# starlingonearth/MASt3R-SLAM-Quality-dualTSDF

Hardware: AMD Instinct MI355X
Metric: SLAM frames/sec (infer+match+TSDF+GN) @512x384 (higher is better)
Workload: dtype bf16

## Files before the change

### include/mslam_hip.h

```cpp
#ifndef MSLAM_HIP_H
#define MSLAM_HIP_H

#include <stddef.h>
#include <stdint.h>

#ifdef __cplusplus
extern "C" {
#endif

#define MSLAM_OK 0
#define MSLAM_EINVAL (-1)
#define MSLAM_EHIP (-2)
#define MSLAM_ENOMEM (-3)
#define MSLAM_ENODEV (-4)

const char* mslam_last_error(void);
int mslam_abi_version(void);
int mslam_device_check(void);


int mslam_iter_proj(const float* rays_img_with_grad, const float* pts_3d_norm,
                    const float* p_init, float* p_new, uint8_t* converged, int b, int h, int w,
                    int n, int max_iter, float lambda_init, float cost_thresh, void* stream);

int mslam_refine_matches(const uint16_t* D11, const uint16_t* D21, const int64_t* p1,
                         int64_t* p1_new, int b, int h, int w, int n, int fdim, int radius,
                         int dilation_max, void* stream);

int mslam_prep_iter_proj(const float* X11, const float* X21, const int64_t* idx_init,
                         float* rays_img_with_grad, float* pts_3d_norm, float* p_init, int b, int h,
                         int w, void* stream);

int mslam_match_occlusion(const float* X11, const float* X21, const float* p, int64_t* p1,
                          uint8_t* valid, int b, int h, int w, float dist_thresh, void* stream);

int mslam_pixel_to_lin(const int64_t* p1, int64_t* idx, int b, int n, int w, void* stream);

size_t mslam_gn_workspace_bytes(int num_poses, int num_edges, int num_points, int local_edges);

int mslam_gauss_newton_rays(float* Twc, const float* Xs, const float* Cs, const int64_t* ii,
                            const int64_t* jj, const int64_t* idx_ii2jj, const uint8_t* valid_match,
                            const float* Q, int num_poses, int num_points, int num_edges,
                            float sigma_ray, float sigma_dist, float C_thresh, float Q_thresh,
                            int max_iter, float delta_thresh, float* dx, void* workspace,
                            size_t workspace_bytes, void* stream);

int mslam_gauss_newton_calib(float* Twc, const float* Xs, const float* Cs, const float* K,
                             const int64_t* ii, const int64_t* jj, const int64_t* idx_ii2jj,
                             const uint8_t* valid_match, const float* Q, int num_poses, int num_points,
                             int num_edges, int height, int width, int pixel_border, float z_eps,
                             float sigma_pixel, float sigma_depth, float C_thresh, float Q_thresh,
                             int max_iter, float delta_thresh, float* dx, void* workspace,
                             size_t workspace_bytes, void* stream);

int mslam_gauss_newton_points(float* Twc, const float* Xs, const float* Cs, const int64_t* ii,
                              const int64_t* jj, const int64_t* idx_ii2jj, const uint8_t* valid_match,
                              const float* Q, int num_poses, int num_points, int num_edges,
                              float sigma_point, float C_thresh, float Q_thresh, int max_iter,
                              float delta_thresh, float* dx, void* workspace, size_t workspace_bytes,
                              void* stream);

int mslam_gn_begin(const int64_t* ii, const int64_t* jj, int num_poses, int num_edges, int num_points,
                   void* workspace, size_t workspace_bytes, void* stream);
int mslam_gn_compact(const float* Xs, const float* Cs, const int64_t* idx_ii2jj, const uint8_t* valid_match,
                     const float* Q, int num_poses, int num_points, int num_edges, int edge_begin,
                     int edge_count, float C_thresh, float Q_thresh, void* workspace, size_t workspace_bytes,
                     void* stream);
int mslam_gn_compact_at(const float* Xs, const float* Cs, const int64_t* idx_ii2jj, const uint8_t* valid_match,
                        const float* Q, int num_poses, int num_points, int num_edges, int edge_begin, int edge_count,
                        int slot_begin, int range_count, float C_thresh, float Q_thresh, void* workspace,
                        size_t workspace_bytes, void* stream);
int mslam_gn_accumulate(int kind, const float* Twc, const float* K, int num_poses, int num_points,
                        int num_edges, int edge_begin, int edge_count, float sigma_a, float sigma_b,
                        int height, int width, int pixel_border, float z_eps, float* Hs, float* gs,
                        void* workspace, size_t workspace_bytes, void* stream);
int mslam_gn_solve_retract(const float* Hs, const float* gs, int num_poses, int num_edges,
                           int num_points, float* Twc, float* dx, float delta_thresh, void* workspace,
                           size_t workspace_bytes, void* stream);
int mslam_gn_status(int* status4, int num_poses, int num_edges, int num_points, void* workspace,
                    size_t workspace_bytes, void* stream);

int mslam_sim3_act(const float* T, const float* X, float* Y, int num_poses, long long pts_per_pose,
                   int broadcast_pose, void* stream);
int mslam_sim3_op(int op, const float* A, const float* B, float* out, int n, int bcast_a, int bcast_b,
                  void* stream);

size_t mslam_tsdf_table_bytes(uint64_t capacity);
int mslam_tsdf_table_init(void* table, size_t table_bytes, uint64_t capacity, void* stream);

size_t mslam_tsdf_integrate_workspace_bytes(int n_points, double voxel_size, double trunc, double step_scale);
int mslam_tsdf_integrate(void* table, uint64_t capacity, const float* points_world, const double* conf,
                         const float* cam_origin, int n_points, double voxel_size, double trunc,
                         double max_weight, double step_scale, int shard_id, int num_shards,
                         void* workspace, size_t workspace_bytes, void* stream);

int mslam_tsdf_rehash(void* old_table, uint64_t old_capacity, void* new_table, uint64_t new_capacity, void* stream);
int mslam_tsdf_header(void* table, uint64_t capacity, uint32_t* out8_host, void* stream);

int mslam_tsdf_dump(void* table, uint64_t capacity, int64_t* keys, double* tsdf, double* weight,
                    uint32_t max_out, void* stream);

int mslam_tsdf_query(void* table, uint64_t capacity, const float* points, int n, double voxel_size,
                     double min_weight, double* value, double* grad, uint8_t* status, void* stream);

int mslam_tsdf_pose_step(void* table, uint64_t capacity, const float* points, const float* conf, int n,
                         float* pose, int points_in_camera_frame, double voxel_size, double min_weight,
                         double lambda, double damping, int update_pose, double* H_out, double* b_out,
                         int* used_out, void* workspace, size_t workspace_bytes, void* stream);

int mslam_tsdf_lookup7(void* table, uint64_t capacity, const float* points, int n, const float* pose,
                       double voxel_size, double* out, void* stream);
int mslam_tsdf_query_lookup(const double* lookup, int n, double voxel_size, double min_weight, double* value,
                            double* grad, uint8_t* status, void* stream);
int mslam_tsdf_pose_step_lookup(const double* lookup, const float* points, const float* conf, int n, float* pose,
                                int points_in_camera_frame, double voxel_size, double min_weight, double lambda,
                                double damping, int update_pose, double* H_out, double* b_out, int* used_out,
                                void* workspace, size_t workspace_bytes, void* stream);

size_t mslam_tsdf_mesh_workspace_bytes(uint64_t capacity);
int mslam_tsdf_mesh_keys(void* table, uint64_t capacity, double min_weight, int64_t* sort_keys, void* stream);
int mslam_tsdf_mesh_count(void* table, uint64_t capacity, double min_weight, double level, const int64_t* sorted_keys,
                          const int64_t* order, int32_t* counts, void* workspace, size_t workspace_bytes, void* stream);
int mslam_tsdf_mesh_emit(void* table, uint64_t capacity, double voxel_size, double min_weight, double level,
                         const int64_t* sorted_keys, const int64_t* order, const int64_t* vbase, const int64_t* fbase,
                         void* workspace, size_t workspace_bytes, float* vertices, float* normals, int32_t* faces,
                         int64_t n_vertices, int64_t n_faces, void* stream);
int mslam_tsdf_load(void* table, uint64_t capacity, const int64_t* keys, const double* tsdf, const double* weight,
                    int n, void* stream);

size_t mslam_tsdf_render_workspace_bytes(uint64_t capacity);
int mslam_tsdf_render_blocks(void* table, uint64_t capacity, double min_weight, void* workspace, size_t workspace_bytes,
                             void* stream);
int mslam_tsdf_render(void* table, uint64_t capacity, const float* rays, int h, int w, const float* pose8,
                      double voxel_size, double min_weight, double level, double near, double far, double step, int skip,
                      const void* workspace, size_t workspace_bytes, float* range, float* normal, uint8_t* hit,
                      void* stream);

size_t mslam_tsdf_color_bytes(uint64_t capacity);
int mslam_tsdf_color_init(void* color, size_t color_bytes, uint64_t capacity, void* stream);
int mslam_tsdf_integrate_color(void* table, uint64_t capacity, void* color, const float* points_world,
                               const double* conf, const float* rgb, const float* cam_origin, int n_points,
                               double voxel_size, double trunc, double step_scale, void* stream);
int mslam_tsdf_color_rehash(void* old_table, uint64_t old_capacity, const void* old_color, void* new_table,
                            uint64_t new_capacity, void* new_color, void* stream);
int mslam_tsdf_color_dump(void* table, uint64_t capacity, const void* color, const int64_t* keys, int n, uint64_t* sums,
                          void* stream);
int mslam_tsdf_color_load(void* table, uint64_t capacity, void* color, const int64_t* keys, const uint64_t* sums, int n,
                          void* stream);
int mslam_tsdf_color_sample(void* table, uint64_t capacity, const void* color, const float* points, int n, int image_w,
                            double voxel_size, double default_r, double default_g, double default_b, float* out_rgb,
                            uint8_t* out_count, void* stream);

int mslam_mast3r_create(void** handle_out, const int* cfg9_host, void* const* weight_ptrs_host,
                        const long long* weight_numels_host, int n_weights, void* stream);
int mslam_mast3r_destroy(void* handle);
size_t mslam_mast3r_workspace_bytes(void* handle, int batch, int H, int W);

int mslam_mast3r_encode(void* handle, const float* img, int batch, int H, int W, float* feat_out,
                        void* workspace, size_t workspace_bytes, void* stream);

int mslam_mast3r_decode(void* handle, const float* feat1, const float* feat2, int batch, int H, int W,
                        float* X1, float* C1, float* D1, float* Q1, float* X2, float* C2, float* D2,
                        float* Q2, float* dec_last1, float* dec_last2, void* workspace,
                        size_t workspace_bytes, void* stream);

size_t mslam_track_workspace_bytes(int n_points);
int mslam_track_pose(int use_calib, float* T_rel, const float* Xf, const float* Xk, const int64_t* idx_f2k,
                     const float* Qk, const uint8_t* valid, int n_points, const float* K, int width,
                     int height, float sigma_a, float sigma_b, float huber, int pixel_border, float z_eps,
                     int first_iter, int max_iters, float rel_error, float delta_norm, void* status_out, void* workspace,
                     size_t workspace_bytes, void* stream);

size_t mslam_track_prepare_workspace_bytes(int n_points);
int mslam_track_prepare(const int64_t* idx_f2k, const uint8_t* valid_match, const float* Qff, const float* Qkf,
                        const float* Cf_sum, float inv_nf, const float* Ck_sum, float inv_nk, float C_conf, float Q_conf,
                        int n_points, const float* T_WCk, const float* T_WCf, float* Qk, float* Ck_avg,
                        uint8_t* valid_opt, uint8_t* valid_kf, float* T_rel, void* workspace, size_t workspace_bytes,
                        void* stream);
int mslam_track_verdict(const void* prepare_workspace, const void* status, int n_points, float* verdict6, void* stream);
int mslam_track_fuse(const float* T_WCk, const float* T_rel, const float* Xkf, const float* Ckf, const float* X_canon,
                     const float* C, int n_points, float* T_WCf, float* X_new, float* C_new, void* stream);

int mslam_gemm_bf16(const void* A, const void* W, const float* bias, const void* residual_f32, void* out,
                    int M, int N, int K, int act, int out_is_bf16, void* stream);
int mslam_gemm_tile_override(int M, int N, int K, int cfg);
int mslam_gemm_profile_begin(int M, int N, int K, int max_samples);
int mslam_gemm_profile_end(double* avg_us, double* min_us, int* samples);
int mslam_conv2d_nhwc_bf16(const void* in, const void* W, const float* bias, const void* residual_bf16,
                           void* out_bf16, int B, int H, int Wd, int Cin, int Cout, int ks, int stride,
                           int relu_in, int act, void* stream);
int mslam_attention_bf16(const void* Q, const void* K, const void* VT, void* O, int batch, int heads,
                         int nq, int nk, void* stream);
int mslam_layernorm_f32(const float* x, const float* w, const float* b, void* out_bf16, float* out_f32,
                        int rows, int D, float eps, void* stream);

size_t mslam_tsdf_local_workspace_bytes(int n_points);
int mslam_tsdf_local_build(const float* X_world, const float* C, const float* origin, const float* xyz_min,
                           const float* xyz_max, int n_points, int nx, int ny, int nz, double voxel_size,
                           double trunc, float min_confidence, float* tsdf, float* weights, void* workspace,
                           size_t workspace_bytes, void* stream);
int mslam_tsdf_local_raycast(const float* tsdf, int nx, int ny, int nz, const float* xyz_min,
                             const float* xyz_max, const float* X_original, const int64_t* sel_pix, int n_sel,
                             int n_samples, float max_displacement, float* surf, uint8_t* hit, void* stream);

int mslam_quality_reduce_grid(const float* x, const float* y, const uint8_t* valid, int h, int w, int ps, int mode,
                              double c_thr, double q_thr, float* out, void* stream);
int mslam_quality_classify(const float* delta_cov, const float* r, const float* u, int n, float thr_zr, float thr_zu,
                           float thr_dc, int64_t* cls, float* pri, void* stream);

int mslam_room_pair(const float* ki, const float* kj, int batch, int h, int w, int n_frames, double fx, double fy,
                    double cx, double cy, double noise, const double* Wm_3x24, const double* phase_24, float* X1,
                    float* C1, float* D1, float* Q1, float* X2, float* C2, float* D2, float* Q2, void* stream);

int mslam_remap_bilinear_u8(const uint8_t* src, int src_h, int src_w, int channels, const float* mapx,
                            const float* mapy, uint8_t* dst, int dst_h, int dst_w, void* stream);

int mslam_gemm_f64(const void* A, int a_is_f32, const void* B, int b_is_f32, int b_transposed, const double* centre,
                   const double* bias, double* out, int M, int N, int K, void* stream);

int mslam_asmk_aggregate(const float* des, const float* centroids, const int64_t* assign, const int64_t* uniq_words,
                         uint32_t* sig_out, int n_des, int m_assign, int dim, int n_uniq, int n_centroids, void* stream);
int mslam_asmk_search(const int32_t* entry_word, const uint32_t* entry_sig, const int32_t* img_start, int n_images,
                      const int32_t* q_words, const uint32_t* q_sig, int n_q, int sig_words, float similarity_threshold,
                      float alpha, double* scores, void* stream);

#ifdef __cplusplus
}
#endif
#endif
```

### mast3r-slam-quality-dualtsdf_amd/csrc/tracker.hip

```cpp
#include "common.h"
#include "sim3.h"

namespace mslam {

constexpr int kTAcc = 36;

struct TrackState {
  int done;
  int iters;
  int chol_fail;
  float old_cost;
  float last_cost;
  float last_delta_norm;
  float pad0, pad1;
};

struct TrackParams {
  float inv_sigma_a, inv_sigma_b;
  float huber_k;
  const float* K;
  float border_lo, border_hi_u, border_hi_v, z_eps;
  int width;
};

__device__ __forceinline__ float huber_k(float r, float k) {
  const float a = fabsf(r);
  return a < k ? 1.0f : k / a;
}

template <unsigned NZ>
__device__ __forceinline__ void taccum_row(float (&acc)[kTAcc], const float (&x)[7], float w, float err) {
  const float we = w * err;
  int l = 0;
#pragma unroll
  for (int n = 0; n < 7; n++) {
    const float wx = w * x[n];
#pragma unroll
    for (int m = 0; m <= n; m++) {
      if (((NZ >> n) & 1u) && ((NZ >> m) & 1u)) acc[l] = fmaf(wx, x[m], acc[l]);
      l++;
    }
    if ((NZ >> n) & 1u) acc[28 + n] = fmaf(we, x[n], acc[28 + n]);
  }
  acc[35] = fmaf(we, err, acc[35]);
}

template <int CALIB>
__global__ __launch_bounds__(256) void track_accum_kernel(const TrackState* __restrict__ st,
                                                          const float* __restrict__ T,
                                                          const float* __restrict__ Xf, const float* __restrict__ Xk,
                                                          const int64_t* __restrict__ idx, const float* __restrict__ Qk,
                                                          const uint8_t* __restrict__ valid, int n, TrackParams P,
                                                          float* __restrict__ partial) {
  if (st->done) return;
  const Sim3f Tr = sim3_load(T);
  float R[9];
  quat_to_mat(Tr.q, R);
  float acc[kTAcc];
#pragma unroll
  for (int l = 0; l < kTAcc; l++) acc[l] = 0.0f;
  for (int k = blockIdx.x * 256 + threadIdx.x; k < n; k += gridDim.x * 256) {
    const long long j = idx[k];
    const float xf0 = Xf[j * 3], xf1 = Xf[j * 3 + 1], xf2 = Xf[j * 3 + 2];
    const float xk0 = Xk[(size_t)k * 3], xk1 = Xk[(size_t)k * 3 + 1], xk2 = Xk[(size_t)k * 3 + 2];
    const float p0 = Tr.s * (R[0] * xf0 + R[1] * xf1 + R[2] * xf2) + Tr.t[0];
    const float p1 = Tr.s * (R[3] * xf0 + R[4] * xf1 + R[5] * xf2) + Tr.t[1];
    const float p2 = Tr.s * (R[6] * xf0 + R[7] * xf1 + R[8] * xf2) + Tr.t[2];
    const float vq = valid[k] ? sqrtf(Qk[k]) : 0.0f;
    if constexpr (CALIB == 0) {
      const float nk = sqrtf(xk0 * xk0 + xk1 * xk1 + xk2 * xk2), nk_inv = 1.0f / nk;
      const float n2 = p0 * p0 + p1 * p1 + p2 * p2;
      const float np = sqrtf(n2), np_inv = 1.0f / np;
      const float r0 = p0 * np_inv, r1 = p1 * np_inv, r2 = p2 * np_inv;
      const float e0 = r0 - xk0 * nk_inv, e1 = r1 - xk1 * nk_inv, e2 = r2 - xk2 * nk_inv, e3 = np - nk;
      const float sa = P.inv_sigma_a * vq, sb = P.inv_sigma_b * vq;
      const float w0 = huber_k(sa * e0, P.huber_k) * sa * sa, w1 = huber_k(sa * e1, P.huber_k) * sa * sa;
      const float w2 = huber_k(sa * e2, P.huber_k) * sa * sa, w3 = huber_k(sb * e3, P.huber_k) * sb * sb;
      const float n3 = np_inv / n2;
      const float dxx = np_inv - p0 * p0 * n3, dyy = np_inv - p1 * p1 * n3, dzz = np_inv - p2 * p2 * n3;
      const float dxy = -p0 * p1 * n3, dxz = -p0 * p2 * n3, dyz = -p1 * p2 * n3;
      { const float x[7] = {dxx, dxy, dxz, 0.0f, r2, -r1, 0.0f}; taccum_row<0b0110111>(acc, x, w0, e0); }
      { const float x[7] = {dxy, dyy, dyz, -r2, 0.0f, r0, 0.0f}; taccum_row<0b0101111>(acc, x, w1, e1); }
      { const float x[7] = {dxz, dyz, dzz, r1, -r0, 0.0f, 0.0f}; taccum_row<0b0011111>(acc, x, w2, e2); }
      { const float x[7] = {r0, r1, r2, 0.0f, 0.0f, 0.0f, np}; taccum_row<0b1000111>(acc, x, w3, e3); }
    } else {
      const float Pfx = P.K[0], Pfy = P.K[4], Pcx = P.K[2], Pcy = P.K[5];
      const float uk = (float)(k % P.width), vk = (float)(k / P.width);
      const bool valid_meas = xk2 > P.z_eps;
      const float lzk = valid_meas ? logf(xk2) : 0.0f;
      const float zinv = 1.0f / p2;
      const float u = Pfx * p0 * zinv + Pcx, v = Pfy * p1 * zinv + Pcy;
      const bool valid_z = p2 > P.z_eps;
      const bool valid_p = (u > P.border_lo) && (u < P.border_hi_u) && (v > P.border_lo) && (v < P.border_hi_v) && valid_z;
      const float lz = valid_z ? logf(p2) : 0.0f;
      const float gate = (valid_p && valid_meas) ? vq : 0.0f;
      const float e0 = u - (valid_meas ? uk : 0.0f), e1 = v - (valid_meas ? vk : 0.0f), e2 = lz - lzk;
      const float sa = P.inv_sigma_a * gate, sb = P.inv_sigma_b * gate;
      const float w0 = huber_k(sa * e0, P.huber_k) * sa * sa, w1 = huber_k(sa * e1, P.huber_k) * sa * sa;
      const float w2 = huber_k(sb * e2, P.huber_k) * sb * sb;
      const float xz = p0 * zinv, yz = p1 * zinv;
      if (gate > 0.0f) {
        { const float x[7] = {Pfx * zinv, 0.0f, -Pfx * xz * zinv, -Pfx * xz * yz, Pfx * (1.0f + xz * xz), -Pfx * yz, 0.0f};
          taccum_row<0b0111101>(acc, x, w0, e0); }
        { const float x[7] = {0.0f, Pfy * zinv, -Pfy * yz * zinv, -Pfy * (1.0f + yz * yz), Pfy * xz * yz, Pfy * xz, 0.0f};
          taccum_row<0b0111110>(acc, x, w1, e1); }
        { const float x[7] = {0.0f, 0.0f, zinv, yz, -xz, 0.0f, 1.0f}; taccum_row<0b1011100>(acc, x, w2, e2); }
      }
    }
  }
  __shared__ float red[4][kTAcc];
  const int lane = threadIdx.x & 63, wid = threadIdx.x >> 6;
#pragma unroll
  for (int l = 0; l < kTAcc; l++) {
    const float s = wave_sum(acc[l]);
    if (lane == 0) red[wid][l] = s;
  }
  __syncthreads();
  if (threadIdx.x < kTAcc)
    partial[(size_t)blockIdx.x * kTAcc + threadIdx.x] =
        (red[0][threadIdx.x] + red[1][threadIdx.x]) + (red[2][threadIdx.x] + red[3][threadIdx.x]);
}

__global__ __launch_bounds__(64) void track_solve_kernel(TrackState* __restrict__ st, const float* __restrict__ partial,
                                                         int nblk, float* __restrict__ T, float rel_thresh,
                                                         float delta_thresh) {
  if (st->done) return;
  __shared__ double s[kTAcc];
  const int t = threadIdx.x;
  if (t < kTAcc) {
    double a = 0.0;
    for (int k = 0; k < nblk; k++) a += (double)partial[(size_t)k * kTAcc + t];
    s[t] = a;
  }
  __syncthreads();
  if (t != 0) return;
  double H[7][7], g[7];
  int l = 0;
  for (int n = 0; n < 7; n++)
    for (int m = 0; m <= n; m++) { H[n][m] = s[l]; H[m][n] = s[l]; l++; }
  for (int n = 0; n < 7; n++) g[n] = -s[28 + n];
  const float cost = (float)(0.5 * s[35]);
  double L[7][7];
  bool fail = false;
  for (int j = 0; j < 7 && !fail; j++) {
    double d = H[j][j];
    for (int k = 0; k < j; k++) d -= L[j][k] * L[j][k];
    if (!(d > 0.0)) { fail = true; break; }
    L[j][j] = sqrt(d);
    for (int i = j + 1; i < 7; i++) {
      double v = H[i][j];
      for (int k = 0; k < j; k++) v -= L[i][k] * L[j][k];
      L[i][j] = v / L[j][j];
    }
  }
  st->iters += 1;
  st->last_cost = cost;
  if (fail) { st->chol_fail = 1; st->done = 1; return; }
  double y[7], x[7];
  for (int i = 0; i < 7; i++) { double v = g[i]; for (int k = 0; k < i; k++) v -= L[i][k] * y[k]; y[i] = v / L[i][i]; }
  for (int i = 6; i >= 0; i--) { double v = y[i]; for (int k = i + 1; k < 7; k++) v -= L[k][i] * x[k]; x[i] = v / L[i][i]; }
  float tau[7];
  double nn = 0.0;
  for (int i = 0; i < 7; i++) { tau[i] = (float)x[i]; nn += (double)tau[i] * tau[i]; }
  sim3_store(T, sim3_unit(sim3_retr(tau, sim3_load(T))));
  const float delta_norm = (float)sqrt(nn);
  st->last_delta_norm = delta_norm;
  const float old = st->old_cost;
  const float rel_dec = fabsf((old - cost) / old);
  if (rel_dec < rel_thresh || delta_norm < delta_thresh) st->done = 1;
  st->old_cost = cost;
}

__global__ void track_init_kernel(TrackState* st) {
  st->done = 0; st->iters = 0; st->chol_fail = 0; st->old_cost = INFINITY; st->last_cost = 0.0f;
  st->last_delta_norm = 0.0f; st->pad0 = st->pad1 = 0.0f;
}

__device__ __host__ inline size_t prep_partials_bytes(int n) { return (((size_t)((n + 255) / 256) * 8) + 255) & ~(size_t)255; }

__global__ __launch_bounds__(256) void track_prep_kernel(
    const int64_t* __restrict__ idx, const uint8_t* __restrict__ vmatch, const float* __restrict__ Qff,
    const float* __restrict__ Qkf, const float* __restrict__ Cf_sum, float inv_nf, const float* __restrict__ Ck_sum,
    float inv_nk, float C_conf, float Q_conf, int n, const float* __restrict__ T_WCk, const float* __restrict__ T_WCf,
    float* __restrict__ Qk, float* __restrict__ Ck_avg, uint8_t* __restrict__ valid_opt, uint8_t* __restrict__ valid_kf,
    float* __restrict__ T_rel, int2* __restrict__ partial, uint8_t* __restrict__ hit) {
  const int k = blockIdx.x * 256 + threadIdx.x;
  if (k == 0) {
    const Sim3f Ti = sim3_unit(sim3_inv(sim3_load(T_WCk)));
    sim3_store(T_rel, sim3_unit(sim3_mul(Ti, sim3_load(T_WCf))));
  }
  bool opt = false, kf = false;
  if (k < n) {
    const long long j = idx[k];
    const bool vm = vmatch[k] != 0;
    const float q = sqrtf(Qff[j] * Qkf[k]);
    const float cf = Cf_sum[j] * inv_nf;
    const float ck = Ck_sum[k] * inv_nk;
    const bool vq = q > Q_conf;
    opt = vm && (cf > C_conf) && (ck > C_conf) && vq;
    kf = vm && vq;
    Qk[k] = q;
    Ck_avg[k] = ck;
    valid_opt[k] = opt ? 1 : 0;
    valid_kf[k] = kf ? 1 : 0;
    if (vm) hit[j] = 1;
  }
  __shared__ int red[4][2];
  const int c_opt = __popcll(__ballot(opt)), c_kf = __popcll(__ballot(kf));
  if ((threadIdx.x & 63) == 0) { red[threadIdx.x >> 6][0] = c_opt; red[threadIdx.x >> 6][1] = c_kf; }
  __syncthreads();
  if (threadIdx.x == 0)
    partial[blockIdx.x] = make_int2(red[0][0] + red[1][0] + red[2][0] + red[3][0], red[0][1] + red[1][1] + red[2][1] + red[3][1]);
}

__global__ __launch_bounds__(1024) void track_verdict_kernel(const int2* __restrict__ partial, const uint8_t* __restrict__ hit,
                                                             const int* __restrict__ status, int n, float* __restrict__ out) {
  const int t = threadIdx.x;
  int c[3] = {0, 0, 0};
  const int nblk = (n + 255) / 256;
  for (int b = t; b < nblk; b += 1024) { const int2 p = partial[b]; c[0] += p.x; c[1] += p.y; }
  const int n16 = n >> 4;
  for (int v = t; v < n16; v += 1024) {
    const uint4 w = reinterpret_cast<const uint4*>(hit)[v];
    c[2] += __popc(w.x) + __popc(w.y) + __popc(w.z) + __popc(w.w);
  }
  for (int v = (n16 << 4) + t; v < n; v += 1024) c[2] += hit[v];
  __shared__ int red[16][3];
#pragma unroll
  for (int q = 0; q < 3; q++) {
    int s = c[q];
#pragma unroll
    for (int off = 32; off > 0; off >>= 1) s += __shfl_down(s, off, 64);
    if ((t & 63) == 0) red[t >> 6][q] = s;
  }
  __syncthreads();
  if (t != 0) return;
  int tot[3] = {0, 0, 0};
  for (int w = 0; w < 16; w++) { tot[0] += red[w][0]; tot[1] += red[w][1]; tot[2] += red[w][2]; }
  const float inv_n = 1.0f / (float)n;
  out[0] = (float)tot[0] * inv_n;
  out[1] = (float)status[1];
  out[2] = (float)status[2];
  out[3] = (float)tot[1] * inv_n;
  out[4] = (float)tot[2] * inv_n;
  out[5] = (float)status[0];
}

__global__ __launch_bounds__(256) void track_fuse_kernel(const float* __restrict__ T_WCk, const float* __restrict__ T_rel,
                                                         const float* __restrict__ Xkf, const float* __restrict__ Ckf,
                                                         const float* __restrict__ Xc, const float* __restrict__ Cc, int n,
                                                         float* __restrict__ T_WCf, float* __restrict__ Xn,
                                                         float* __restrict__ Cn) {
  const int k = blockIdx.x * 256 + threadIdx.x;
  const Sim3f Tr = sim3_load(T_rel);
  if (k == 0) sim3_store(T_WCf, sim3_unit(sim3_mul(sim3_load(T_WCk), Tr)));
  if (k >= n) return;
  const float x[3] = {Xkf[(size_t)k * 3], Xkf[(size_t)k * 3 + 1], Xkf[(size_t)k * 3 + 2]};
  float y[3];
  sim3_act(Tr, x, y);
  const float c = Cc[k], cn = Ckf[k], den = c + cn;
#pragma unroll
  for (int d = 0; d < 3; d++) Xn[(size_t)k * 3 + d] = ((c * Xc[(size_t)k * 3 + d]) + (cn * y[d])) / den;
  Cn[k] = den;
}

}

using namespace mslam;

extern "C" size_t mslam_track_workspace_bytes(int n_points) {
  (void)n_points;
  return 256 + sizeof(float) * kTAcc * 1024;
}

extern "C" int mslam_track_pose(int use_calib, float* T_rel, const float* Xf, const float* Xk, const int64_t* idx_f2k,
                                const float* Qk, const uint8_t* valid, int n_points, const float* K, int width,
                                int height, float sigma_a, float sigma_b, float huber, int pixel_border, float z_eps,
                                int first_iter, int max_iters, float rel_error, float delta_norm, void* status_out,
                                void* workspace, size_t workspace_bytes, void* stream) {
  MSLAM_REQUIRE(n_points > 0 && max_iters >= 0 && first_iter >= 0, "track_pose: bad sizes");
  MSLAM_REQUIRE(T_rel && Xf && Xk && idx_f2k && Qk && valid && workspace, "track_pose: null pointer");
  MSLAM_REQUIRE(!use_calib || (K && width > 0 && height > 0), "track_pose: calib needs K, width, height");
  MSLAM_REQUIRE(workspace_bytes >= mslam_track_workspace_bytes(n_points), "track_pose: workspace too small");
  hipStream_t s = (hipStream_t)stream;
  TrackState* st = (TrackState*)workspace;
  float* partial = (float*)((char*)workspace + 256);
  int nblk = (n_points + 256 * 8 - 1) / (256 * 8);
  if (nblk > 1024) nblk = 1024;
  if (nblk < 1) nblk = 1;
  TrackParams P = {};
  P.inv_sigma_a = 1.0f / sigma_a; P.inv_sigma_b = 1.0f / sigma_b; P.huber_k = huber;
  P.width = width > 0 ? width : 1;
  if (use_calib) {
    P.K = K;
    P.border_lo = (float)pixel_border; P.border_hi_u = (float)(width - 1 - pixel_border);
    P.border_hi_v = (float)(height - 1 - pixel_border); P.z_eps = z_eps;
  }
  if (first_iter == 0) hipLaunchKernelGGL(track_init_kernel, dim3(1), dim3(1), 0, s, st);
  for (int it = first_iter; it < max_iters; it++) {
    if (use_calib)
      hipLaunchKernelGGL(track_accum_kernel<1>, dim3(nblk), dim3(256), 0, s, st, T_rel, Xf, Xk, idx_f2k, Qk, valid,
                         n_points, P, partial);
    else
      hipLaunchKernelGGL(track_accum_kernel<0>, dim3(nblk), dim3(256), 0, s, st, T_rel, Xf, Xk, idx_f2k, Qk, valid,
                         n_points, P, partial);
    hipLaunchKernelGGL(track_solve_kernel, dim3(1), dim3(64), 0, s, st, partial, nblk, T_rel, rel_error, delta_norm);
  }
  MSLAM_LAUNCH_CHECK("track_pose");
  if (status_out)
    return check_hip(hipMemcpyAsync(status_out, st, sizeof(TrackState), hipMemcpyDeviceToDevice, s), "track status");
  return MSLAM_OK;
}

extern "C" size_t mslam_track_prepare_workspace_bytes(int n_points) {
  return 256 + prep_partials_bytes(n_points) + (((size_t)n_points + 255) & ~(size_t)255);
}

extern "C" int mslam_track_prepare(const int64_t* idx_f2k, const uint8_t* valid_match, const float* Qff,
                                   const float* Qkf, const float* Cf_sum, float inv_nf, const float* Ck_sum,
                                   float inv_nk, float C_conf, float Q_conf, int n_points, const float* T_WCk,
                                   const float* T_WCf, float* Qk, float* Ck_avg, uint8_t* valid_opt, uint8_t* valid_kf,
                                   float* T_rel, void* workspace, size_t workspace_bytes, void* stream) {
  MSLAM_REQUIRE(n_points > 0, "track_prepare: bad sizes");
  MSLAM_REQUIRE(idx_f2k && valid_match && Qff && Qkf && Cf_sum && Ck_sum && T_WCk && T_WCf && Qk && Ck_avg && valid_opt &&
                    valid_kf && T_rel && workspace, "track_prepare: null pointer");
  MSLAM_REQUIRE(workspace_bytes >= mslam_track_prepare_workspace_bytes(n_points), "track_prepare: workspace too small");
  hipStream_t s = (hipStream_t)stream;
  MSLAM_REQUIRE(((uintptr_t)workspace & 15) == 0, "track_prepare: workspace must be 16-byte aligned");
  uint8_t* hit = (uint8_t*)workspace + 256 + prep_partials_bytes(n_points);
  int rc = check_hip(hipMemsetAsync(hit, 0, (size_t)n_points, s), "track_prepare: memset");
  if (rc) return rc;
  hipLaunchKernelGGL(track_prep_kernel, dim3((n_points + 255) / 256), dim3(256), 0, s, idx_f2k, valid_match, Qff, Qkf,
                     Cf_sum, inv_nf, Ck_sum, inv_nk, C_conf, Q_conf, n_points, T_WCk, T_WCf, Qk, Ck_avg, valid_opt,
                     valid_kf, T_rel, (int2*)((char*)workspace + 256), hit);
  MSLAM_LAUNCH_CHECK("track_prepare");
  return MSLAM_OK;
}

extern "C" int mslam_track_verdict(const void* prepare_workspace, const void* status, int n_points, float* verdict6,
                                   void* stream) {
  MSLAM_REQUIRE(prepare_workspace && status && verdict6 && n_points > 0, "track_verdict: bad arguments");
  const char* ws = (const char*)prepare_workspace;
  hipLaunchKernelGGL(track_verdict_kernel, dim3(1), dim3(1024), 0, (hipStream_t)stream, (const int2*)(ws + 256),
                     (const uint8_t*)(ws + 256 + prep_partials_bytes(n_points)), (const int*)status, n_points, verdict6);
  MSLAM_LAUNCH_CHECK("track_verdict");
  return MSLAM_OK;
}

extern "C" int mslam_track_fuse(const float* T_WCk, const float* T_rel, const float* Xkf, const float* Ckf,
                                const float* X_canon, const float* C, int n_points, float* T_WCf, float* X_new,
                                float* C_new, void* stream) {
  MSLAM_REQUIRE(n_points > 0, "track_fuse: bad sizes");
  MSLAM_REQUIRE(T_WCk && T_rel && Xkf && Ckf && X_canon && C && T_WCf && X_new && C_new, "track_fuse: null pointer");
  hipLaunchKernelGGL(track_fuse_kernel, dim3((n_points + 255) / 256), dim3(256), 0, (hipStream_t)stream, T_WCk, T_rel, Xkf,
                     Ckf, X_canon, C, n_points, T_WCf, X_new, C_new);
  MSLAM_LAUNCH_CHECK("track_fuse");
  return MSLAM_OK;
}
```

### mast3r-slam-quality-dualtsdf_amd/mast3r_slam/tracker.py

```python
import copy
import time

import numpy as np
import torch

import mslam_hip as _m
from lietorch_hip import Sim3
from mast3r_slam.config import config
from mast3r_slam.geometry import act_Sim3, constrain_points_to_ray, point_to_ray_dist
from mast3r_slam.mast3r_utils import mast3r_match_asymmetric


class _Pending:
    __slots__ = ("frame", "init_T", "prev_idx", "prev_shadow", "stash", "base", "shadow", "slot", "job", "verdict",
                 "event", "quality", "T_WCf", "T_CkCf", "T_WCk", "Xkf", "Ckf", "Qkf", "Qff", "status", "n_points", "replayed",
                 "kind", "vals", "new_kf")


class FrameTracker:
    IN_PLACE_MODES = ("indep_conf",)

    def __init__(self, model, frames, device):
        self.cfg = config["tracking"]
        self.model = model
        self.keyframes = frames
        self.device = device
        self.reset_idx_f2k()
        self.N_SLOTS = 4
        self._slots = [dict(ws=None, status=None, host=None, prep=None) for _ in range(self.N_SLOTS)]
        self._slot = 0
        self._shadow = None
        self.quality_service = None
        self.last_kf_value = None
        self.verdict_wait_s = 0.0

    def reset_idx_f2k(self):
        self.idx_f2k = None

    def track(self, frame):
        h = self.track_begin(frame)
        self.track_resolve(h)
        return self.track_finish(h)

    def track_begin(self, frame):
        h = _Pending()
        h.frame, h.replayed = frame, False
        h.init_T, h.prev_idx, h.prev_shadow = frame.T_WC, self.idx_f2k, self._shadow
        h.stash = getattr(frame, "decoded", None)
        stored = self.keyframes.last_keyframe()
        keyframe = self._shadow if self._shadow is not None else stored
        idx_f2k, valid_match_k, Xff, Cff, Qff, Xkf, Ckf, Qkf = mast3r_match_asymmetric(
            self.model, frame, keyframe, idx_i2j_init=self.idx_f2k)
        self.idx_f2k = idx_f2k.clone()
        idx_f2k = idx_f2k[0]
        valid_match_k = valid_match_k[0]
        frame.update_pointmap(Xff, Cff)

        use_calib = config["use_calib"]
        img_size = frame.img.shape[-2:]
        K = keyframe.K if use_calib else None
        T_WCk = stored.T_WC
        Xf, Xk = frame.X_canon, keyframe.X_canon
        if use_calib:
            Xf = constrain_points_to_ray(img_size, Xf[None], K).squeeze(0)
            Xk = constrain_points_to_ray(img_size, Xk[None], K).squeeze(0)
        self._idx = idx_f2k

        h.slot = self._slot
        self._slot = (self._slot + 1) % self.N_SLOTS
        self._cur = h
        Qk, Ck, valid_opt, valid_kf, T_rel = self._prepare(h, frame, keyframe, idx_f2k, valid_match_k, Qff, Qkf,
                                                           T_WCk, frame.T_WC)
        T_WCf, T_CkCf, status = self._run_async(use_calib, Xf, Xk, None, T_WCk, Qk, valid_opt, K if use_calib else None,
                                                img_size if use_calib else None, chunked=True, T_rel=T_rel, pose=False)
        h.job, h.T_WCk = getattr(self, "_job", None), T_WCk
        h.status = status
        self._post_verdict(h)
        h.quality = None
        if self.quality_service is not None and not use_calib:
            h.quality = dict(Xf=Xf, idx=idx_f2k, Xk=Xk, valid_kf=valid_kf.view(-1), Ck=Ck.view(-1), Qk=Qk.view(-1),
                             kf_id=int(len(self.keyframes) - 1), frame_id=int(keyframe.frame_id), H=int(img_size[0]),
                             W=int(img_size[1]))
        h.base, h.Xkf, h.Ckf, h.Qkf, h.Qff = keyframe, Xkf, Ckf, Qkf, Qff
        self._apply(h, T_WCf, T_CkCf)
        return h

    def _prepare(self, h, frame, keyframe, idx_f2k, valid_match_k, Qff, Qkf, T_WCk, T_WCf):
        n = int(keyframe.X_canon.shape[0])
        dev = idx_f2k.device
        L = _m.lib()
        sl = self._slots[h.slot]
        need = L.mslam_track_prepare_workspace_bytes(n)
        if sl.get("prep") is None or sl["prep"].numel() < need:
            sl["prep"] = torch.empty(need, dtype=torch.uint8, device=dev)
        Qk = torch.empty((n, 1), dtype=torch.float32, device=dev)
        Ck = torch.empty((n, 1), dtype=torch.float32, device=dev)
        valid_opt = torch.empty((n, 1), dtype=torch.bool, device=dev)
        valid_kf = torch.empty((n, 1), dtype=torch.bool, device=dev)
        T_rel = torch.empty(8, dtype=torch.float32, device=dev)
        idx_c, vm_c = idx_f2k.contiguous(), valid_match_k.contiguous()
        Qff_c, Qkf_c = Qff.contiguous(), Qkf.contiguous()
        Cf_c, Ck_c = frame.C.contiguous(), keyframe.C.contiguous()
        Tk_c, Tf_c = T_WCk.data.reshape(8).contiguous(), T_WCf.data.reshape(8).contiguous()
        _m.require_dtype(idx_c, torch.int64, "idx_f2k")
        _m.require_dtype(vm_c, torch.bool, "valid_match_k")
        inv_nf = float(np.float32(1.0) / np.float32(frame.N))
        inv_nk = float(np.float32(1.0) / np.float32(keyframe.N))
        rc = L.mslam_track_prepare(_m.ptr(idx_c), _m.ptr(vm_c), _m.ptr(Qff_c), _m.ptr(Qkf_c), _m.ptr(Cf_c), inv_nf,
                                   _m.ptr(Ck_c), inv_nk, float(self.cfg["C_conf"]), float(self.cfg["Q_conf"]), n,
                                   _m.ptr(Tk_c), _m.ptr(Tf_c), _m.ptr(Qk), _m.ptr(Ck), _m.ptr(valid_opt),
                                   _m.ptr(valid_kf), _m.ptr(T_rel), _m.ptr(sl["prep"]), sl["prep"].numel(),
                                   _m.stream_ptr())
        _m.check(rc, "track_prepare")
        h.n_points = n
        return Qk, Ck, valid_opt, valid_kf, T_rel

    def _post_verdict(self, h):
        sl = self._slots[h.slot]
        dev = torch.empty(6, dtype=torch.float32, device=h.status.device)
        rc = _m.lib().mslam_track_verdict(_m.ptr(sl["prep"]), _m.ptr(h.status), int(h.n_points), _m.ptr(dev),
                                          _m.stream_ptr())
        _m.check(rc, "track_verdict")
        if sl["host"] is None:
            sl["host"] = torch.empty(6, dtype=torch.float32).pin_memory()
        sl["host"].copy_(dev, non_blocking=True)
        h.event = torch.cuda.Event()
        h.event.record()
        h.verdict = sl["host"]

    def _apply(self, h, T_WCf, T_CkCf):
        h.T_CkCf = T_CkCf
        base = h.base
        shadow = copy.copy(base)
        shadow._in_store, shadow._replaced_by = False, None
        T_WCk = h.T_WCk
        if config["tracking"]["filtering_mode"] == "weighted_pointmap" and base.N > 0:
            n = int(base.X_canon.shape[0])
            dev = base.X_canon.device
            T_out = torch.empty((1, 8), dtype=torch.float32, device=dev)
            X_new, C_new = torch.empty_like(base.X_canon), torch.empty_like(base.C)
            Tk_c, Tr_c = T_WCk.data.reshape(8).contiguous(), T_CkCf.data.reshape(8).contiguous()
            Xkf_c, Ckf_c = h.Xkf.contiguous(), h.Ckf.contiguous()
            Xc_c, Cc_c = base.X_canon.contiguous(), base.C.contiguous()
            assert X_new.is_contiguous() and C_new.is_contiguous()
            rc = _m.lib().mslam_track_fuse(_m.ptr(Tk_c), _m.ptr(Tr_c), _m.ptr(Xkf_c), _m.ptr(Ckf_c), _m.ptr(Xc_c),
                                           _m.ptr(Cc_c), n, _m.ptr(T_out), _m.ptr(X_new), _m.ptr(C_new), _m.stream_ptr())
            _m.check(rc, "track_fuse")
            if T_WCf is None:
                T_WCf = Sim3(T_out)
            shadow.X_canon, shadow.C = X_new, C_new
            shadow.N, shadow.N_updates = base.N + 1, base.N_updates + 1
        else:
            if T_WCf is None:
                T_WCf = T_WCk * T_CkCf
            Xkk = T_CkCf.act(h.Xkf)
            if config["tracking"]["filtering_mode"] in self.IN_PLACE_MODES:
                shadow.X_canon, shadow.C = shadow.X_canon.clone(), shadow.C.clone()
            shadow.update_pointmap(Xkk, h.Ckf)
        h.T_WCf = T_WCf
        h.frame.T_WC = T_WCf
        h.shadow = shadow
        self._shadow = shadow

    def track_resolve(self, h):
        t_wait = time.perf_counter()
        h.event.synchronize()
        self.verdict_wait_s += time.perf_counter() - t_wait
        v = h.verdict.tolist()
        if v[0] >= self.cfg["min_match_frac"] and int(v[5]) == 0 and int(v[2]) == 0 and int(v[1]) < int(self.cfg["max_iters"]):
            self._cur = h
            _, T_CkCf, h.status = self._run_rest()
            self._post_verdict(h)
            h.event.synchronize()
            v = h.verdict.tolist()
            stale = h.shadow
            later = self._shadow if self._shadow is not stale else None
            self._apply(h, None, T_CkCf)
            stale._replaced_by = h.shadow
            if later is not None:
                self._shadow = later
            h.replayed = True
        h.vals = v
        self.last_iters = int(v[1])
        skip = v[0] < self.cfg["min_match_frac"] or int(v[2]) != 0
        h.kind = "skip" if skip else "ok"
        h.new_kf = (not skip) and min(float(v[3]), float(v[4])) < self.cfg["match_frac_thresh"]
        return h.kind

    def track_finish(self, h):
        frame = h.frame
        if h.kind == "skip":
            frame.T_WC = h.init_T
            if self._shadow is h.shadow:
                self._shadow = self._live(h.prev_shadow)
            return False, [], True
        if h.quality is not None:
            q = h.quality
            T_CkCf = h.T_CkCf

            def residual_map(q=q, T=T_CkCf):
                Xf_g = q["Xf"][q["idx"]]
                rd_k = point_to_ray_dist(q["Xk"], jacobian=False)
                rd_f = point_to_ray_dist(act_Sim3(T, Xf_g, jacobian=False), jacobian=False)
                vec = T.data.view(-1, 8)
                w = vec[..., 6].clamp(-1.0, 1.0).abs()
                return {"r_pix": torch.linalg.norm(rd_k - rd_f, dim=1), "t_norm": vec[..., :3].norm(dim=-1).mean(),
                        "theta": (2.0 * torch.arccos(w)).mean()}

            self.quality_service.submit({
                "kf_id": q["kf_id"], "frame_id": q["frame_id"], "H": q["H"], "W": q["W"], "valid_kf": q["valid_kf"],
                "Ck": q["Ck"], "Qk": q["Qk"], "lazy": residual_map, "keep": (q["Xf"], q["idx"], q["Xk"], T_CkCf.data)})
        keyframe = h.shadow
        keyframe.T_WC = self.keyframes.last_keyframe().T_WC
        self.keyframes[len(self.keyframes) - 1] = keyframe
        keyframe._in_store = True
        if self._shadow is h.shadow:
            self._shadow = None
        match_frac_k, unique_frac_f = float(h.vals[3]), float(h.vals[4])
        self.last_kf_value = min(match_frac_k, unique_frac_f)
        new_kf = h.new_kf
        if new_kf:
            self.reset_idx_f2k()
            self._shadow = None
        return (new_kf, [keyframe.X_canon, keyframe.get_average_conf(), frame.X_canon, frame.get_average_conf(),
                         h.Qkf, h.Qff], False)

    @staticmethod
    def _live(shadow):
        while shadow is not None and getattr(shadow, "_replaced_by", None) is not None:
            shadow = shadow._replaced_by
        return None if shadow is None or getattr(shadow, "_in_store", False) else shadow

    def rollback(self, h):
        self.idx_f2k, self._shadow = h.prev_idx, self._live(h.prev_shadow)
        f = h.frame
        f.T_WC, f.X_canon, f.C, f.N, f.N_updates = h.init_T, None, None, 0, 0
        if h.stash is not None:
            f.decoded = h.stash

    def get_points_poses(self, frame, keyframe, idx_f2k, img_size, use_calib, K=None):
        Xf, Xk = frame.X_canon, keyframe.X_canon
        Cf, Ck = frame.get_average_conf(), keyframe.get_average_conf()
        meas_k = valid_meas_k = None
        if use_calib:
            Xf = constrain_points_to_ray(img_size, Xf[None], K).squeeze(0)
            Xk = constrain_points_to_ray(img_size, Xk[None], K).squeeze(0)
        self._idx = idx_f2k
        return Xf, Xk, frame.T_WC, keyframe.T_WC, Cf[idx_f2k], Ck, meas_k, valid_meas_k

    def _run(self, use_calib, Xf, Xk, T_WCf, T_WCk, Qk, valid, K, img_size, idx=None):
        T_WCf_new, T_CkCf, status = self._run_async(use_calib, Xf, Xk, T_WCf, T_WCk, Qk, valid, K, img_size, idx)
        st = status.cpu()
        self.last_iters = int(st[1])
        return T_WCf_new, T_CkCf, int(st[2]) == 0

    FIRST_CHUNK = 8

    def _run_async(self, use_calib, Xf, Xk, T_WCf, T_WCk, Qk, valid, K, img_size, idx=None, chunked=False, T_rel=None,
                   pose=True):
        cfg = self.cfg
        dev = Xf.device
        idx = self._idx if idx is None else idx
        n = Xk.shape[0]
        if T_rel is None:
            T_rel = (T_WCk.inv() * T_WCf).data.reshape(8).contiguous().clone()
        L = _m.lib()
        need = L.mslam_track_workspace_bytes(n)
        cur = getattr(self, "_cur", None)
        sl = self._slots[cur.slot if cur is not None else 0]
        if sl["ws"] is None or sl["ws"].numel() < need:
            sl["ws"] = torch.empty(need, dtype=torch.uint8, device=dev)
            sl["status"] = torch.zeros(8, dtype=torch.int32, device=dev)
        h, w = (int(img_size[0]), int(img_size[1])) if img_size is not None else (0, 0)
        sa, sb = (cfg["sigma_pixel"], cfg["sigma_depth"]) if use_calib else (cfg["sigma_ray"], cfg["sigma_dist"])
        Xf_c, Xk_c, idx_c = Xf.contiguous(), Xk.contiguous(), idx.contiguous()
        Qk_c, valid_c = Qk.reshape(-1).contiguous(), valid.reshape(-1).contiguous()
        K_c = K.contiguous() if use_calib else None
        self._job = dict(args=(int(use_calib), _m.ptr(T_rel), _m.ptr(Xf_c), _m.ptr(Xk_c), _m.ptr(idx_c), _m.ptr(Qk_c),
                               _m.ptr(valid_c), n, _m.ptr(K_c) if use_calib else 0,
                               w, h, float(sa), float(sb), float(cfg["huber"]), int(cfg["pixel_border"]),
                               float(cfg["depth_eps"])),
                         keep=(T_rel, Xf_c, Xk_c, idx_c, Qk_c, valid_c, K_c), T_rel=T_rel, T_WCk=T_WCk, slot=sl, pose=pose)
        last = min(self.FIRST_CHUNK, int(cfg["max_iters"])) if chunked else int(cfg["max_iters"])
        return self._enqueue(self._job, 0, last)

    def _enqueue(self, job, first, last):
        cfg, sl = self.cfg, job["slot"]
        rc = _m.lib().mslam_track_pose(*job["args"], int(first), int(last), float(cfg["rel_error"]),
                                       float(cfg["delta_norm"]), _m.ptr(sl["status"]), _m.ptr(sl["ws"]),
                                       sl["ws"].numel(), _m.stream_ptr())
        _m.check(rc, "track_pose")
        T_CkCf = Sim3(job["T_rel"].reshape(1, 8))
        return (job["T_WCk"] * T_CkCf if job["pose"] else None), T_CkCf, sl["status"]

    def _run_rest(self):
        job = self._cur.job if getattr(self, "_cur", None) is not None and self._cur.job is not None else self._job
        return self._enqueue(job, min(self.FIRST_CHUNK, int(self.cfg["max_iters"])), int(self.cfg["max_iters"]))

    def opt_pose_ray_dist_sim3(self, Xf, Xk, T_WCf, T_WCk, Qk, valid, idx=None):
        return self._run(False, Xf, Xk, T_WCf, T_WCk, Qk, valid, None, None, idx)

    def opt_pose_calib_sim3(self, Xf, Xk, T_WCf, T_WCk, Qk, valid, meas_k, valid_meas_k, K, img_size, idx=None):
        return self._run(True, Xf, Xk, T_WCf, T_WCk, Qk, valid, K, img_size, idx)
```

Before: 169.4.

## Fuse tracker accumulate and solve into single last-block-reduces kernel per iteration

Each Gauss-Newton tracking iteration used to launch an accumulation kernel and then a separate single-block solve kernel. These are now merged into one kernel. Blocks write their partial sums, take a ticket from an atomic counter, and the last block to finish reduces the partials in double precision, runs the 7x7 Cholesky solve, updates the pose and state, and resets the ticket. This removes one launch per iteration and the separate init and status-copy launches. In exchange it adds atomic and fence ordering requirements, and the workspace is now zero-initialised so the ticket starts at zero. The old two-kernel path is kept as a reference entry point.

```diff
diff --git a/include/mslam_hip.h b/include/mslam_hip.h
--- a/include/mslam_hip.h
+++ b/include/mslam_hip.h
@@ -170,6 +170,11 @@
                      int height, float sigma_a, float sigma_b, float huber, int pixel_border, float z_eps,
                      int first_iter, int max_iters, float rel_error, float delta_norm, void* status_out, void* workspace,
                      size_t workspace_bytes, void* stream);
+int mslam_track_pose_reference(int use_calib, float* T_rel, const float* Xf, const float* Xk, const int64_t* idx_f2k,
+                               const float* Qk, const uint8_t* valid, int n_points, const float* K, int width,
+                               int height, float sigma_a, float sigma_b, float huber, int pixel_border, float z_eps,
+                               int first_iter, int max_iters, float rel_error, float delta_norm, void* status_out,
+                               void* workspace, size_t workspace_bytes, void* stream);
 
 size_t mslam_track_prepare_workspace_bytes(int n_points);
 int mslam_track_prepare(const int64_t* idx_f2k, const uint8_t* valid_match, const float* Qff, const float* Qkf,
diff --git a/mast3r-slam-quality-dualtsdf_amd/csrc/tracker.hip b/mast3r-slam-quality-dualtsdf_amd/csrc/tracker.hip
--- a/mast3r-slam-quality-dualtsdf_amd/csrc/tracker.hip
+++ b/mast3r-slam-quality-dualtsdf_amd/csrc/tracker.hip
@@ -45,15 +45,11 @@
   acc[35] = fmaf(we, err, acc[35]);
 }
 
-template <int CALIB>
-__global__ __launch_bounds__(256) void track_accum_kernel(const TrackState* __restrict__ st,
-                                                          const float* __restrict__ T,
-                                                          const float* __restrict__ Xf, const float* __restrict__ Xk,
-                                                          const int64_t* __restrict__ idx, const float* __restrict__ Qk,
-                                                          const uint8_t* __restrict__ valid, int n, TrackParams P,
-                                                          float* __restrict__ partial) {
-  if (st->done) return;
-  const Sim3f Tr = sim3_load(T);
+template <int CALIB, bool WRITE_THROUGH = false>
+__device__ __forceinline__ void track_block_row(const Sim3f& Tr, const float* __restrict__ Xf,
+                                                const float* __restrict__ Xk, const int64_t* __restrict__ idx,
+                                                const float* __restrict__ Qk, const uint8_t* __restrict__ valid, int n,
+                                                const TrackParams& P, float* partial) {
   float R[9];
   quat_to_mat(Tr.q, R);
   float acc[kTAcc];
@@ -116,9 +112,23 @@
     if (lane == 0) red[wid][l] = s;
   }
   __syncthreads();
-  if (threadIdx.x < kTAcc)
-    partial[(size_t)blockIdx.x * kTAcc + threadIdx.x] =
-        (red[0][threadIdx.x] + red[1][threadIdx.x]) + (red[2][threadIdx.x] + red[3][threadIdx.x]);
+  if (threadIdx.x < kTAcc) {
+    const float v = (red[0][threadIdx.x] + red[1][threadIdx.x]) + (red[2][threadIdx.x] + red[3][threadIdx.x]);
+    float* dst = partial + (size_t)blockIdx.x * kTAcc + threadIdx.x;
+    if constexpr (WRITE_THROUGH) __hip_atomic_store(dst, v, __ATOMIC_RELAXED, __HIP_MEMORY_SCOPE_AGENT);
+    else *dst = v;
+  }
+}
+
+template <int CALIB>
+__global__ __launch_bounds__(256) void track_accum_kernel(const TrackState* __restrict__ st,
+                                                          const float* __restrict__ T,
+                                                          const float* __restrict__ Xf, const float* __restrict__ Xk,
+                                                          const int64_t* __restrict__ idx, const float* __restrict__ Qk,
+                                                          const uint8_t* __restrict__ valid, int n, TrackParams P,
+                                                          float* __restrict__ partial) {
+  if (st->done) return;
+  track_block_row<CALIB>(sim3_load(T), Xf, Xk, idx, Qk, valid, n, P, partial);
 }
 
 __global__ __launch_bounds__(64) void track_solve_kernel(TrackState* __restrict__ st, const float* __restrict__ partial,
@@ -176,6 +186,117 @@
   st->last_delta_norm = 0.0f; st->pad0 = st->pad1 = 0.0f;
 }
 
+constexpr int kTicketByte = 128;
+
+__device__ __forceinline__ double wave_lane_f64(double v, int src) {
+  const int lo = __builtin_amdgcn_readlane(__double2loint(v), src);
+  const int hi = __builtin_amdgcn_readlane(__double2hiint(v), src);
+  return __hiloint2double(hi, lo);
+}
+
+template <int CALIB>
+__global__ __launch_bounds__(256) void track_iter_kernel(TrackState* st, float* T,
+                                                         const float* __restrict__ Xf, const float* __restrict__ Xk,
+                                                         const int64_t* __restrict__ idx, const float* __restrict__ Qk,
+                                                         const uint8_t* __restrict__ valid, int n, TrackParams P,
+                                                         float* partial, unsigned* ticket, int init, float rel_thresh,
+                                                         float delta_thresh, int* status_out) {
+  if (!init && st->done) {
+    if (status_out && blockIdx.x == 0 && threadIdx.x < 8) status_out[threadIdx.x] = reinterpret_cast<const int*>(st)[threadIdx.x];
+    return;
+  }
+  const Sim3f Tr = sim3_load(T);
+  track_block_row<CALIB, true>(Tr, Xf, Xk, idx, Qk, valid, n, P, partial);
+  if (threadIdx.x >= kWave) return;
+  asm volatile("s_waitcnt vmcnt(0)" ::: "memory");
+  unsigned drawn = 0;
+  if (threadIdx.x == 0) drawn = __hip_atomic_fetch_add(ticket, 1u, __ATOMIC_RELAXED, __HIP_MEMORY_SCOPE_AGENT);
+  drawn = (unsigned)__builtin_amdgcn_readfirstlane((int)drawn);
+  const int nblk = gridDim.x;
+  if (drawn != (unsigned)(nblk - 1)) return;
+  __builtin_amdgcn_fence(__ATOMIC_ACQUIRE, "agent");
+  const int t = threadIdx.x;
+  double a = 0.0;
+  if (t < kTAcc) {
+    const float* col = partial + t;
+    int k = 0;
+    for (; k + 32 <= nblk; k += 32) {
+      float v[32];
+#pragma unroll
+      for (int u = 0; u < 32; u++) v[u] = col[(size_t)(k + u) * kTAcc];
+#pragma unroll
+      for (int u = 0; u < 32; u++) a += (double)v[u];
+    }
+    for (; k < nblk; k++) a += (double)col[(size_t)k * kTAcc];
+  }
+  double s[kTAcc];
+#pragma unroll
+  for (int l = 0; l < kTAcc; l++) s[l] = wave_lane_f64(a, l);
+  double g[7];
+#pragma unroll
+  for (int i = 0; i < 7; i++) g[i] = -s[28 + i];
+  const float cost = (float)(0.5 * s[35]);
+  double L[7][7];
+  bool fail = false;
+#pragma unroll
+  for (int j = 0; j < 7; j++) {
+    double d = s[j * (j + 1) / 2 + j];
+#pragma unroll
+    for (int k = 0; k < j; k++) d -= L[j][k] * L[j][k];
+    if (!(d > 0.0)) fail = true;
+    L[j][j] = sqrt(d);
+#pragma unroll
+    for (int i = j + 1; i < 7; i++) {
+      double v = s[i * (i + 1) / 2 + j];
+#pragma unroll
+      for (int k = 0; k < j; k++) v -= L[i][k] * L[j][k];
+      L[i][j] = v / L[j][j];
+    }
+  }
+  TrackState ns;
+  if (init) { ns.done = 0; ns.iters = 0; ns.chol_fail = 0; ns.old_cost = INFINITY; ns.last_cost = 0.0f;
+              ns.last_delta_norm = 0.0f; ns.pad0 = ns.pad1 = 0.0f; }
+  else ns = *st;
+  ns.iters += 1;
+  ns.last_cost = cost;
+  if (fail) {
+    ns.chol_fail = 1; ns.done = 1;
+  } else {
+    double y[7], x[7];
+#pragma unroll
+    for (int i = 0; i < 7; i++) {
+      double v = g[i];
+#pragma unroll
+      for (int k = 0; k < i; k++) v -= L[i][k] * y[k];
+      y[i] = v / L[i][i];
+    }
+#pragma unroll
+    for (int i = 6; i >= 0; i--) {
+      double v = y[i];
+#pragma unroll
+      for (int k = i + 1; k < 7; k++) v -= L[k][i] * x[k];
+      x[i] = v / L[i][i];
+    }
+    float tau[7];
+    double nn = 0.0;
+#pragma unroll
+    for (int i = 0; i < 7; i++) { tau[i] = (float)x[i]; nn += (double)tau[i] * tau[i]; }
+    const Sim3f Tn = sim3_unit(sim3_retr(tau, Tr));
+    if (t == 0) sim3_store(T, Tn);
+    const float delta_norm = (float)sqrt(nn);
+    ns.last_delta_norm = delta_norm;
+    const float old = ns.old_cost;
+    const float rel_dec = fabsf((old - cost) / old);
+    if (rel_dec < rel_thresh || delta_norm < delta_thresh) ns.done = 1;
+    ns.old_cost = cost;
+  }
+  if (t == 0) {
+    *st = ns;
+    if (status_out) *reinterpret_cast<TrackState*>(status_out) = ns;
+    __hip_atomic_store(ticket, 0u, __ATOMIC_RELAXED, __HIP_MEMORY_SCOPE_AGENT);
+  }
+}
+
 __device__ __host__ inline size_t prep_partials_bytes(int n) { return (((size_t)((n + 255) / 256) * 8) + 255) & ~(size_t)255; }
 
 __global__ __launch_bounds__(256) void track_prep_kernel(
@@ -273,17 +394,18 @@
   return 256 + sizeof(float) * kTAcc * 1024;
 }
 
-extern "C" int mslam_track_pose(int use_calib, float* T_rel, const float* Xf, const float* Xk, const int64_t* idx_f2k,
-                                const float* Qk, const uint8_t* valid, int n_points, const float* K, int width,
-                                int height, float sigma_a, float sigma_b, float huber, int pixel_border, float z_eps,
-                                int first_iter, int max_iters, float rel_error, float delta_norm, void* status_out,
-                                void* workspace, size_t workspace_bytes, void* stream) {
+static int track_pose_run(bool fused, int use_calib, float* T_rel, const float* Xf, const float* Xk,
+                          const int64_t* idx_f2k, const float* Qk, const uint8_t* valid, int n_points, const float* K,
+                          int width, int height, float sigma_a, float sigma_b, float huber, int pixel_border, float z_eps,
+                          int first_iter, int max_iters, float rel_error, float delta_norm, void* status_out,
+                          void* workspace, size_t workspace_bytes, void* stream) {
   MSLAM_REQUIRE(n_points > 0 && max_iters >= 0 && first_iter >= 0, "track_pose: bad sizes");
   MSLAM_REQUIRE(T_rel && Xf && Xk && idx_f2k && Qk && valid && workspace, "track_pose: null pointer");
   MSLAM_REQUIRE(!use_calib || (K && width > 0 && height > 0), "track_pose: calib needs K, width, height");
   MSLAM_REQUIRE(workspace_bytes >= mslam_track_workspace_bytes(n_points), "track_pose: workspace too small");
   hipStream_t s = (hipStream_t)stream;
   TrackState* st = (TrackState*)workspace;
+  unsigned* ticket = (unsigned*)((char*)workspace + kTicketByte);
   float* partial = (float*)((char*)workspace + 256);
   int nblk = (n_points + 256 * 8 - 1) / (256 * 8);
   if (nblk > 1024) nblk = 1024;
@@ -296,8 +418,20 @@
     P.border_lo = (float)pixel_border; P.border_hi_u = (float)(width - 1 - pixel_border);
     P.border_hi_v = (float)(height - 1 - pixel_border); P.z_eps = z_eps;
   }
-  if (first_iter == 0) hipLaunchKernelGGL(track_init_kernel, dim3(1), dim3(1), 0, s, st);
+  const bool launches = first_iter < max_iters;
+  if (first_iter == 0 && !(fused && launches)) hipLaunchKernelGGL(track_init_kernel, dim3(1), dim3(1), 0, s, st);
   for (int it = first_iter; it < max_iters; it++) {
+    if (fused) {
+      const int init = it == 0;
+      int* so = it == max_iters - 1 ? (int*)status_out : nullptr;
+      if (use_calib)
+        hipLaunchKernelGGL(track_iter_kernel<1>, dim3(nblk), dim3(256), 0, s, st, T_rel, Xf, Xk, idx_f2k, Qk, valid,
+                           n_points, P, partial, ticket, init, rel_error, delta_norm, so);
+      else
+        hipLaunchKernelGGL(track_iter_kernel<0>, dim3(nblk), dim3(256), 0, s, st, T_rel, Xf, Xk, idx_f2k, Qk, valid,
+                           n_points, P, partial, ticket, init, rel_error, delta_norm, so);
+      continue;
+    }
     if (use_calib)
       hipLaunchKernelGGL(track_accum_kernel<1>, dim3(nblk), dim3(256), 0, s, st, T_rel, Xf, Xk, idx_f2k, Qk, valid,
                          n_points, P, partial);
@@ -307,9 +441,30 @@
     hipLaunchKernelGGL(track_solve_kernel, dim3(1), dim3(64), 0, s, st, partial, nblk, T_rel, rel_error, delta_norm);
   }
   MSLAM_LAUNCH_CHECK("track_pose");
-  if (status_out)
+  if (status_out && !(fused && launches))
     return check_hip(hipMemcpyAsync(status_out, st, sizeof(TrackState), hipMemcpyDeviceToDevice, s), "track status");
   return MSLAM_OK;
+}
+
+extern "C" int mslam_track_pose(int use_calib, float* T_rel, const float* Xf, const float* Xk, const int64_t* idx_f2k,
+                                const float* Qk, const uint8_t* valid, int n_points, const float* K, int width,
+                                int height, float sigma_a, float sigma_b, float huber, int pixel_border, float z_eps,
+                                int first_iter, int max_iters, float rel_error, float delta_norm, void* status_out,
+                                void* workspace, size_t workspace_bytes, void* stream) {
+  return track_pose_run(true, use_calib, T_rel, Xf, Xk, idx_f2k, Qk, valid, n_points, K, width, height, sigma_a, sigma_b,
+                        huber, pixel_border, z_eps, first_iter, max_iters, rel_error, delta_norm, status_out, workspace,
+                        workspace_bytes, stream);
+}
+
+extern "C" int mslam_track_pose_reference(int use_calib, float* T_rel, const float* Xf, const float* Xk,
+                                          const int64_t* idx_f2k, const float* Qk, const uint8_t* valid, int n_points,
+                                          const float* K, int width, int height, float sigma_a, float sigma_b,
+                                          float huber, int pixel_border, float z_eps, int first_iter, int max_iters,
+                                          float rel_error, float delta_norm, void* status_out, void* workspace,
+                                          size_t workspace_bytes, void* stream) {
+  return track_pose_run(false, use_calib, T_rel, Xf, Xk, idx_f2k, Qk, valid, n_points, K, width, height, sigma_a, sigma_b,
+                        huber, pixel_border, z_eps, first_iter, max_iters, rel_error, delta_norm, status_out, workspace,
+                        workspace_bytes, stream);
 }
 
 extern "C" size_t mslam_track_prepare_workspace_bytes(int n_points) {
diff --git a/mast3r-slam-quality-dualtsdf_amd/mast3r_slam/tracker.py b/mast3r-slam-quality-dualtsdf_amd/mast3r_slam/tracker.py
--- a/mast3r-slam-quality-dualtsdf_amd/mast3r_slam/tracker.py
+++ b/mast3r-slam-quality-dualtsdf_amd/mast3r_slam/tracker.py
@@ -269,7 +269,7 @@
         cur = getattr(self, "_cur", None)
         sl = self._slots[cur.slot if cur is not None else 0]
         if sl["ws"] is None or sl["ws"].numel() < need:
-            sl["ws"] = torch.empty(need, dtype=torch.uint8, device=dev)
+            sl["ws"] = torch.zeros(need, dtype=torch.uint8, device=dev)
             sl["status"] = torch.zeros(8, dtype=torch.int32, device=dev)
         h, w = (int(img_size[0]), int(img_size[1])) if img_size is not None else (0, 0)
         sa, sb = (cfg["sigma_pixel"], cfg["sigma_depth"]) if use_calib else (cfg["sigma_ray"], cfg["sigma_dist"])
```

New measurement: 162.6. -4.1%, worse.
